# santi-pdp/segan_pytorch

Measured on NVIDIA H100. Metric: 16384-sample windows/sec (G+D train step), higher is better.
Workload: dtype f16 operands / f32 accumulate (f16 gradient tensors, loss scale 1024)

## Files before the change

### segan_pytorch_b200/csrc/tapgemm_tc.cu

```cuda
#include "common.cuh"
#include <cuda.h>
#include <stdlib.h>

namespace sg {

__device__ __forceinline__ uint32_t smem_u32(const void* p) {
  return static_cast<uint32_t>(__cvta_generic_to_shared(p));
}
__device__ __forceinline__ void mbar_init(uint64_t* bar, uint32_t count) {
  asm volatile("mbarrier.init.shared::cta.b64 [%0], %1;" ::"r"(smem_u32(bar)), "r"(count));
}
__device__ __forceinline__ void mbar_expect_tx(uint64_t* bar, uint32_t bytes) {
  asm volatile("mbarrier.arrive.expect_tx.shared::cta.b64 _, [%0], %1;" ::"r"(smem_u32(bar)), "r"(bytes)
               : "memory");
}
__device__ __forceinline__ void mbar_arrive(uint64_t* bar) {
  asm volatile("mbarrier.arrive.shared::cta.b64 _, [%0];" ::"r"(smem_u32(bar)) : "memory");
}
__device__ __forceinline__ uint32_t mbar_try(uint32_t addr, uint32_t parity) {
  uint32_t done;
  asm volatile(
      "{\n"
      ".reg .pred p;\n"
      "mbarrier.try_wait.parity.shared::cta.b64 p, [%1], %2;\n"
// ... 37 lines not shown
  asm volatile("prefetch.tensormap [%0];" ::"l"(reinterpret_cast<uint64_t>(map)) : "memory");
}
__device__ __forceinline__ void tma_store_3d(const CUtensorMap* map, uint32_t src, int c0, int c1, int c2) {
  asm volatile("cp.async.bulk.tensor.3d.global.shared::cta.bulk_group [%0, {%2, %3, %4}], [%1];"
               ::"l"(reinterpret_cast<uint64_t>(map)), "r"(src), "r"(c0), "r"(c1), "r"(c2)
               : "memory");
}
__device__ __forceinline__ void bulk_commit() { asm volatile("cp.async.bulk.commit_group;" ::: "memory"); }
__device__ __forceinline__ void bulk_wait_read_all() { asm volatile("cp.async.bulk.wait_group.read 0;" ::: "memory"); }
template <int N>
__device__ __forceinline__ void bulk_wait_read() { asm volatile("cp.async.bulk.wait_group.read %0;" ::"n"(N) : "memory"); }
__device__ __forceinline__ void fence_proxy_async_smem() { asm volatile("fence.proxy.async.shared::cta;" ::: "memory"); }
__device__ __forceinline__ void st_shared_u32(uint32_t addr, uint32_t v) {
  asm volatile("st.shared.b32 [%0], %1;" ::"r"(addr), "r"(v) : "memory");
}
__device__ __forceinline__ uint4 ld_shared_v4(uint32_t addr) {
  uint4 v;
  asm volatile("ld.shared.v4.b32 {%0, %1, %2, %3}, [%4];" : "=r"(v.x), "=r"(v.y), "=r"(v.z), "=r"(v.w) : "r"(addr) : "memory");
  return v;
}
__device__ __forceinline__ void red_add_v2(float* addr, float a, float b) {
  asm volatile("red.global.add.v2.f32 [%0], {%1, %2};" ::"l"(addr), "f"(a), "f"(b) : "memory");
}
__device__ __forceinline__ void wgmma_fence() { asm volatile("wgmma.fence.sync.aligned;" ::: "memory"); }
__device__ __forceinline__ void wgmma_commit() { asm volatile("wgmma.commit_group.sync.aligned;" ::: "memory"); }
template <int N>
__device__ __forceinline__ void wgmma_wait() { asm volatile("wgmma.wait_group.sync.aligned %0;" ::"n"(N) : "memory"); }
template <int R>
__device__ __forceinline__ void setmaxnreg_inc() { asm volatile("setmaxnreg.inc.sync.aligned.u32 %0;" ::"n"(R)); }
template <int R>
// ... 86 lines not shown

template <int N, int TA, int TB, bool BF16>
__device__ __forceinline__ void mma_k64(float (&acc)[N / 2], uint64_t da, uint64_t db, uint32_t a_step,
                                        uint32_t b_step, bool first) {
  wgmma_fence();
#pragma unroll
  for (int kk = 0; kk < 4; ++kk)
    wgmma_tile<N, TA, TB, BF16>(acc, da + kk * a_step, db + kk * b_step, (first && kk == 0) ? 0 : 1);
  wgmma_commit();
}

constexpr int STAGES = 4;
constexpr int A_STAGE_BYTES = 128 * 128;
constexpr int B_STAGE_BYTES = 256 * 128;
constexpr int STAGE_BYTES = A_STAGE_BYTES + B_STAGE_BYTES;
constexpr int SMEM_BYTES = STAGES * STAGE_BYTES + 1024  + 256  + 2048 ;
constexpr int SMEM_OPTIN_LIMIT = 232448;
constexpr int OUT_CHUNK_BYTES = 128 * 128;
template <int TN>
struct FSmem {
  static constexpr int RING = 4;
  static constexpr int STAGE_BYTES = A_STAGE_BYTES + TN * 128;
  static constexpr int BUFS = TN == 64 ? 2 : 1;
  static constexpr int BUF_BYTES = (TN == 256 ? 2 : 4) * OUT_CHUNK_BYTES / BUFS;
  static constexpr int STG_OFF = RING * STAGE_BYTES;
  static constexpr int CTL_OFF = STG_OFF + BUFS * BUF_BYTES;
  static constexpr int BYTES = CTL_OFF + 256  + 1024 ;
  static_assert(RING <= STAGES && STAGE_BYTES % 1024 == 0 && BUFS * BUF_BYTES >= 2048, "form-F shared memory");
};
static_assert(FSmem<64>::BYTES <= SMEM_OPTIN_LIMIT, "form-F TN 64 shared memory exceeds the sm_90 opt-in limit");
static_assert(FSmem<128>::BYTES <= SMEM_OPTIN_LIMIT, "form-F TN 128 shared memory exceeds the sm_90 opt-in limit");
static_assert(FSmem<256>::BYTES <= SMEM_OPTIN_LIMIT, "form-F TN 256 shared memory exceeds the sm_90 opt-in limit");
constexpr int NUM_THREADS = 384;
constexpr int PRODUCER_REGS = 40, CONSUMER_REGS = 232;

struct TapRangesTC {
  int k_lo[NTAP], k_hi[NTAP], n_lo[NTAP], n_hi[NTAP];
};

struct FTcParams {
  int a0_c, kc, nc, a_halo;
  int d_lo, d_hi;
  TapRangesTC tr;
// ... 114 lines not shown
    t.m_rel = 0;
    t.m0 = p.m_lo1;
    t.TR = p.TR1; t.TB = p.TB1; t.seg = 1;
  }
  return t;
}

__device__ __forceinline__ int f_mod(int x, int mod, int mask) { return mask >= 0 ? (x & mask) : (x % mod); }

__device__ __forceinline__ uint32_t pack2(float x, float y, int dtype) {
  if (dtype == SG_F16) return pack_half2_sat(x, y);
  __nv_bfloat162 h = __floats2bfloat162_rn(x, y);
  return *reinterpret_cast<uint32_t*>(&h);
}

__device__ __forceinline__ void f_store2(const FTcParams& p, float& x, float& y, int64_t o, int n_abs, bool atomic,
                                         int64_t o2, int64_t o2mirror) {
  if (p.out_dtype == SG_F32) {
    float* dst = reinterpret_cast<float*>(p.out) + o;
    if (atomic) red_add_v2(dst, x, y);
    else *reinterpret_cast<float2*>(dst) = make_float2(x, y);
    return;
  }
  float s0 = 0.f, s1 = 0.f;
  if (p.slope != nullptr) {
    const float* sp = p.slope + f_mod(n_abs, p.slope_mod, p.slope_mask);
    s0 = __ldg(sp); s1 = __ldg(sp + 1);
    if (p.out2 == nullptr) {
      x = x > 0.f ? x : s0 * x;
      y = y > 0.f ? y : s1 * y;
    }
  }
  *reinterpret_cast<uint32_t*>(reinterpret_cast<uint16_t*>(p.out) + o) = pack2(x, y, p.out_dtype);
  if (p.out2 != nullptr) {
    const uint32_t a = pack2(x > 0.f ? x : s0 * x, y > 0.f ? y : s1 * y, p.out_dtype);
    *reinterpret_cast<uint32_t*>(reinterpret_cast<uint16_t*>(p.out2) + o2) = a;
    if (o2mirror >= 0) *reinterpret_cast<uint32_t*>(reinterpret_cast<uint16_t*>(p.out2) + o2mirror) = a;
  }
}

__device__ __forceinline__ float round_as_stored(float x, int dtype) {
  if (dtype == SG_F16) return __half2float(__float2half_rn(x));
  if (dtype == SG_BF16) return __bfloat162float(__float2bfloat16_rn(x));
  return x;
}

template <int TN>
__device__ __forceinline__ void f_epilogue(const FTcParams& p, float (&acc)[TN / 2], const FTile& t, int n0, int ks,
                                           int ctid, float* colstat) {
  const int lane = ctid & 31, cw = ctid >> 5;
  const int out_buf_rows = p.out_rows + 2 * p.out_halo;
  const int out2_buf_rows = p.out_rows + 2 * p.out2_halo;
  const int col0 = n0 - p.n_lo + p.out_col0 + 2 * (lane & 3);
  int64_t obase[2], o2base[2], o2mirror[2];
  bool valid[2];
#pragma unroll
  for (int h = 0; h < 2; ++h) {
    const int r = cw * 16 + (lane >> 2) + 8 * h;
    const int tb = r / t.TR, tr = r - tb * t.TR;
    const int b = t.b0 + tb, m = t.m0 + tr;
    valid[h] = (tb < t.TB) && (b < p.batch) && (m < p.m_hi);
    obase[h] = ((int64_t)b * out_buf_rows + (m + p.out_halo)) * p.out_ld + col0;
    o2base[h] = 0; o2mirror[h] = -1;
    if (p.out2 != nullptr) {
      const int64_t rb = (int64_t)b * out2_buf_rows + p.out2_halo;
      o2base[h] = (rb + m) * p.out_ld + col0;
      if (p.out2_halo > 0) {
        int mm = 0;
        bool has = false;
        if (m >= 1 && m <= p.out2_halo) { mm = -m; has = true; }
        else if (m >= p.out_rows - 1 - p.out2_halo && m <= p.out_rows - 2) { mm = 2 * (p.out_rows - 1) - m; has = true; }
        if (has) o2mirror[h] = (rb + mm) * p.out_ld + col0;
      }
    }
  }
  const bool add_bias = p.bias != nullptr && ks == 0;
  const bool atomic = p.ksplit > 1;
#pragma unroll
  for (int j = 0; j < TN / 8; ++j) {
    const int c = 8 * j + 2 * (lane & 3);
    float bx = 0.f, by = 0.f;
    if (add_bias) {
      const float* bp = p.bias + f_mod(n0 + c, p.bias_mod, p.bias_mask);
      bx = __ldg(bp); by = __ldg(bp + 1);
    }
    float sx = 0.f, sy = 0.f, qx = 0.f, qy = 0.f;
#pragma unroll
    for (int h = 0; h < 2; ++h) {
      float x = acc[4 * j + 2 * h] + bx, y = acc[4 * j + 2 * h + 1] + by;
      if (valid[h]) {
        f_store2(p, x, y, obase[h] + 8 * j, n0 + c, atomic, o2base[h] + 8 * j, o2mirror[h] >= 0 ? o2mirror[h] + 8 * j : -1);
        x = round_as_stored(x, p.out_dtype);
        y = round_as_stored(y, p.out_dtype);
        sx += x; sy += y; qx += x * x; qy += y * y;
      }
    }
    if (p.stats != nullptr) {
#pragma unroll
      for (int o = 4; o < 32; o <<= 1) {
        sx += __shfl_xor_sync(0xffffffffu, sx, o);
        sy += __shfl_xor_sync(0xffffffffu, sy, o);
        qx += __shfl_xor_sync(0xffffffffu, qx, o);
        qy += __shfl_xor_sync(0xffffffffu, qy, o);
      }
      if (lane < 4) {
        atomicAdd(colstat + c, sx);
        atomicAdd(colstat + c + 1, sy);
        atomicAdd(colstat + 256 + c, qx);
        atomicAdd(colstat + 256 + c + 1, qy);
      }
    }
  }
}

template <bool F16>
__device__ __forceinline__ uint32_t pack2_t(float x, float y) {
  if constexpr (F16) return pack_half2_sat(x, y);
  __nv_bfloat162 h = __floats2bfloat162_rn(x, y);
  return *reinterpret_cast<uint32_t*>(&h);
}

template <int TN, bool F16, int MODE>
__device__ __forceinline__ void f_epilogue_tma_body(const FTcParams& p, const float (&acc)[TN / 2], const FTile& t,
                                                    int n0, int ctid, uint32_t buf, const CUtensorMap* tmO,
                                                    const CUtensorMap* tmO2) {
  constexpr bool two = MODE == 2;
  constexpr bool act_in_place = MODE == 1;
  const int lane = ctid & 31, cw = ctid >> 5;
  const int b0 = t.b0, m0 = t.m0;
  const bool add_bias = p.bias != nullptr;
  const uint32_t row_off = (uint32_t)(cw * 16 + (lane >> 2)) * 128u + 4u * (lane & 3);
  const int sw = lane >> 2;
  const int halo2 = p.out2_halo;
  const bool mirror_tile = two && halo2 > 0 &&
                           ((m0 <= halo2 && m0 + t.TR > 1) || (m0 + t.TR > p.out_rows - 1 - halo2 && m0 <= p.out_rows - 2));
  constexpr int NQ = TN / 64;
  constexpr int CH = FSmem<TN>::BUF_BYTES / OUT_CHUNK_BYTES;
  constexpr int QPR = two ? CH / 2 : CH;
  const int c_rel = n0 - p.n_lo, m_rel = t.m_rel;
#pragma unroll
// ... 30 lines not shown
        if constexpr (two) st_shared_u32(slot + OUT_CHUNK_BYTES + off, pack2_t<F16>(x > 0.f ? x : s0 * x, y > 0.f ? y : s1 * y));
      }
    }
    if (qi != QPR - 1 && q != NQ - 1) continue;
    fence_proxy_async_smem();
    consumer_bar_sync();
    if (ctid == 0) {
#pragma unroll
      for (int k = 0; k <= qi; ++k) {
        const uint32_t src = buf + (uint32_t)(two ? 2 * k : k) * OUT_CHUNK_BYTES;
        const int cq = c_rel + 64 * (q - qi + k);
        tma_store_3d(tmO, src, cq, m_rel, b0);
        if constexpr (two) tma_store_3d(tmO2, src + OUT_CHUNK_BYTES, cq, m_rel, b0);
      }
      bulk_commit();
    }
    if (mirror_tile) {
      const int rows = t.TR * t.TB;
      const int out2_buf_rows = p.out_rows + 2 * halo2;
      for (int idx = ctid; idx < rows * 8 * (qi + 1); idx += 256) {
        const int k = idx / (rows * 8), rk = idx - k * rows * 8;
        const int r = rk >> 3, kb = rk & 7;
        const int tb = r / t.TR, tr = r - tb * t.TR;
        const int b = b0 + tb, m = m0 + tr;
        if (b >= p.batch || m >= p.m_hi) continue;
        int mm;
        if (m >= 1 && m <= halo2) mm = -m;
        else if (m >= p.out_rows - 1 - halo2 && m <= p.out_rows - 2) mm = 2 * (p.out_rows - 1) - m;
        else continue;
        const uint32_t src = buf + (uint32_t)(2 * k + 1) * OUT_CHUNK_BYTES;
        const uint4 v = ld_shared_v4(src + (uint32_t)r * 128u + (uint32_t)((kb ^ (r & 7)) << 4));
        const int64_t o = ((int64_t)b * out2_buf_rows + halo2 + mm) * p.out_ld + p.out_col0 + c_rel +
                          64 * (q - qi + k) + 8 * kb;
        *reinterpret_cast<uint4*>(reinterpret_cast<uint16_t*>(p.out2) + o) = v;
      }
    }
  }
}

template <int TN>
__device__ __forceinline__ void f_epilogue_tma(const FTcParams& p, const float (&acc)[TN / 2], const FTile& t, int n0,
                                               int ctid, uint32_t buf, const CUtensorMap* tmO,
                                               const CUtensorMap* tmO2) {
  const int mode = p.out2 != nullptr ? 2 : (p.slope != nullptr ? 1 : 0);
  if (p.out_dtype == SG_F16) {
    if (mode == 2) f_epilogue_tma_body<TN, true, 2>(p, acc, t, n0, ctid, buf, tmO, tmO2);
    else if (mode == 1) f_epilogue_tma_body<TN, true, 1>(p, acc, t, n0, ctid, buf, tmO, tmO2);
    else f_epilogue_tma_body<TN, true, 0>(p, acc, t, n0, ctid, buf, tmO, tmO2);
  } else {
    if (mode == 2) f_epilogue_tma_body<TN, false, 2>(p, acc, t, n0, ctid, buf, tmO, tmO2);
    else if (mode == 1) f_epilogue_tma_body<TN, false, 1>(p, acc, t, n0, ctid, buf, tmO, tmO2);
    else f_epilogue_tma_body<TN, false, 0>(p, acc, t, n0, ctid, buf, tmO, tmO2);
  }
}

template <int TN, bool BF16>
__global__ void __launch_bounds__(NUM_THREADS, 1)
tapgemm_f_tc(const __grid_constant__ CUtensorMap tmA0, const __grid_constant__ CUtensorMap tmA1,
             const __grid_constant__ CUtensorMap tmW, const __grid_constant__ CUtensorMap tmO,
             const __grid_constant__ CUtensorMap tmO2, const __grid_constant__ CUtensorMap tmA0s1,
             const __grid_constant__ CUtensorMap tmA1s1, const __grid_constant__ CUtensorMap tmOs1,
             const FTcParams p) {
  extern __shared__ uint8_t smem_raw[];
  uint8_t* smem = reinterpret_cast<uint8_t*>((reinterpret_cast<uintptr_t>(smem_raw) + 1023) & ~uintptr_t(1023));
  using L = FSmem<TN>;
  SharedCtl* ctl = reinterpret_cast<SharedCtl*>(smem + L::CTL_OFF);
  float* colstat = reinterpret_cast<float*>(smem + L::STG_OFF);
  const int wg = threadIdx.x >> 7;

  if (threadIdx.x == 0) {
    prefetch_tmap(&tmA0); prefetch_tmap(&tmA1); prefetch_tmap(&tmW);
    if (p.tma_out) {
      prefetch_tmap(&tmO);
      if (p.out2 != nullptr) prefetch_tmap(&tmO2);
    }
    if (p.TR1 > 0) {
      prefetch_tmap(&tmA0s1); prefetch_tmap(&tmA1s1);
      if (p.tma_out) prefetch_tmap(&tmOs1);
    }
    for (int s = 0; s < L::RING; ++s) { mbar_init(&ctl->full[s], 1); mbar_init(&ctl->empty[s], 2); }
    fence_barrier_init();
  }
  if (p.stats != nullptr)
    for (int c = threadIdx.x; c < 512; c += NUM_THREADS) colstat[c] = 0.f;
  __syncthreads();

  const int total_tiles = p.m_tiles * p.n_tiles * p.ksplit;
  const uint32_t b_bytes = (uint32_t)TN * 128u;
  PieceIter it;
  it.init(p, p.m_tiles, total_tiles, blockIdx.x, gridDim.x);
  Piece pc;

  if (wg == 0) {
    setmaxnreg_dec<PRODUCER_REGS>();
    if (threadIdx.x == 0) {
      int stage = 0; uint32_t phase = 0;
      while (it.next(p, pc)) {
        const int ks = p.ksplit == 1 ? 0 : pc.rest % p.ksplit;
        const int nt = p.ksplit == 1 ? pc.rest : pc.rest / p.ksplit;
// ... 38 lines not shown
          }
          step += nk;
        }
      }
    }
    return;
  }

  setmaxnreg_inc<CONSUMER_REGS>();
  const int ctid = threadIdx.x - 128;
  const int cwg = wg - 1;
  const bool wg_leader = (threadIdx.x & 127) == 0;
  const uint32_t smem0 = smem_u32(smem);
  int stage = 0; uint32_t phase = 0;
  int stat_nt = -1;
  auto flush_stats = [&](int nt_done) {
    consumer_bar_sync();
    const int n0s = p.n_lo + nt_done * p.TN;
    double* o = p.stats + (int64_t)(blockIdx.x % SG_STAT_SLICES) * 2 * p.nc;
    for (int c = ctid; c < p.TN; c += 256) {
      atomicAdd(o + n0s + c, (double)colstat[c]);
      atomicAdd(o + p.nc + n0s + c, (double)colstat[256 + c]);
      colstat[c] = 0.f;
      colstat[256 + c] = 0.f;
    }
    consumer_bar_sync();
  };
  const bool tl_on = (p.dbg & (1 << 20)) && ctid == 0 && blockIdx.x < TL_CTAS;
  int tl_i = 0;
  unsigned long long* tl = g_tc_timeline + (blockIdx.x < TL_CTAS ? blockIdx.x : 0) * TL_SLOTS;
  if (tl_on) { for (int i = 0; i < TL_SLOTS; ++i) tl[i] = 0; tl[tl_i++] = gtime_ns(); }

  int staged = 0;
  float acc[TN / 2];
  while (it.next(p, pc)) {
    const int ks = p.ksplit == 1 ? 0 : pc.rest % p.ksplit;
    const int nt = p.ksplit == 1 ? pc.rest : pc.rest / p.ksplit;
    const int n0 = p.n_lo + nt * p.TN;
    const bool partial = pc.tile >= it.dp_end;
    if (p.stats != nullptr && nt != stat_nt) {
      if (stat_nt >= 0) flush_stats(stat_nt);
      stat_nt = nt;
    }
    const int nsteps = pc.ke - pc.kb;
    if (nsteps == 0) {
#pragma unroll
      for (int j = 0; j < TN / 2; ++j) acc[j] = 0.f;
    }
    int prev = 0;
    for (int i = 0; i < nsteps; ++i) {
      mbar_wait(&ctl->full[stage], phase);
      const uint32_t sa = smem0 + (uint32_t)stage * L::STAGE_BYTES;
      mma_k64<TN, 0, 0, BF16>(acc, make_smem_desc(sa + (uint32_t)cwg * 8192u, 16, 1024),
                        make_smem_desc(sa + A_STAGE_BYTES, 16, 1024), 2, 2, i == 0);
      wgmma_wait<1>();
      if (i > 0 && wg_leader) mbar_arrive(&ctl->empty[prev]);
      prev = stage;
      if (++stage == L::RING) { stage = 0; phase ^= 1; }
    }
    wgmma_wait<0>();
    if (nsteps > 0 && wg_leader) mbar_arrive(&ctl->empty[prev]);
    if (tl_on && tl_i < TL_SLOTS - 1) tl[tl_i++] = gtime_ns();

    if (!partial) {
      if (p.tma_out) {
        const uint32_t buf = smem0 + L::STG_OFF + (uint32_t)(staged++ % L::BUFS) * L::BUF_BYTES;
        const FTile t = f_tile(p, pc.mt);
        f_epilogue_tma<TN>(p, acc, t, n0, ctid, buf, t.seg ? &tmOs1 : &tmO, &tmO2);
      } else f_epilogue<TN>(p, acc, f_tile(p, pc.mt), n0, ks, ctid, colstat);
      if (tl_on && tl_i < TL_SLOTS - 1) tl[tl_i++] = gtime_ns();
      continue;
    }
    constexpr int64_t SLOT_F2 = 128 * 256 / 2;
    float2* myslot = reinterpret_cast<float2*>(p.sk_ws) + (int64_t)blockIdx.x * SLOT_F2 + ctid;
#pragma unroll
    for (int j = 0; j < TN / 4; ++j) __stcg(myslot + j * 256, make_float2(acc[2 * j], acc[2 * j + 1]));
    if (tl_on && tl_i < TL_SLOTS - 1) tl[tl_i++] = gtime_ns();
    const int slot = pc.tile - it.dp_end;
    unsigned int* cnt = p.sk_cnt + slot * 8 + (ctid >> 5);
    __threadfence();
    __syncwarp();
    unsigned int old = 0;
    if ((ctid & 31) == 0) old = atomicAdd(cnt, 1u);
    old = __shfl_sync(0xffffffffu, old, 0);
    if (old + 1u == (unsigned int)p.sk_split) {
      __threadfence();
#pragma unroll
      for (int j = 0; j < TN / 2; ++j) acc[j] = 0.f;
      const float2* base0 = reinterpret_cast<const float2*>(p.sk_ws) + (int64_t)slot * p.sk_split * SLOT_F2 + ctid;
      for (int sp = 0; sp < p.sk_split; ++sp) {
#pragma unroll
        for (int j = 0; j < TN / 4; ++j) {
          const float2 t = __ldcg(base0 + sp * SLOT_F2 + j * 256);
          acc[2 * j] += t.x; acc[2 * j + 1] += t.y;
        }
      }
      f_epilogue<TN>(p, acc, f_tile(p, pc.mt), n0, 0, ctid, colstat);
      __syncwarp();
      if ((ctid & 31) == 0) *cnt = 0u;
      if (tl_on && tl_i < TL_SLOTS - 1) tl[tl_i++] = gtime_ns() | (1ull << 63);
    }
  }
  if (tl_on && tl_i < TL_SLOTS) tl[tl_i++] = gtime_ns();
  if (p.stats != nullptr && stat_nt >= 0) flush_stats(stat_nt);
  if (p.tma_out && ctid == 0) bulk_wait_read_all();
}

struct WTcParams {
  int a0_c, kc, nc, a_halo;
  int d_lo, d_hi;
  TapRangesTC tr;
  float* dw; int dw_tap0;
  int g_rows, batch, ksplit;
  int PR, PB;
  int n_tiles, k_tiles;
  int row_chunks, b_chunks;
  const float* out_scale;
};

// ... 197 lines not shown
static int num_sms() {
  static int n = 0;
  if (n == 0) {
    int dev = 0;
    cudaGetDevice(&dev);
    cudaDeviceGetAttribute(&n, cudaDevAttrMultiProcessorCount, dev);
    if (n <= 0) n = NUM_SMS;
  }
  return n;
}

template <typename K>
static int launch_persistent(K kern, int grid, const CUtensorMap& t0, const CUtensorMap& t1, const CUtensorMap& t2,
                             const void* params, cudaStream_t st);

int tapgemm_f_tc_launch(const sg_tapgemm_f* q, cudaStream_t st) {
  FTcParams p;
  p.a0_c = q->a0_c; p.kc = q->kc; p.nc = q->nc; p.a_halo = q->a_halo;
  p.d_lo = q->d_lo; p.d_hi = q->d_hi;
  for (int i = 0; i < NTAP; ++i) {
    p.tr.k_lo[i] = q->tap_k_lo[i]; p.tr.k_hi[i] = q->tap_k_hi[i];
    p.tr.n_lo[i] = q->tap_n_lo[i]; p.tr.n_hi[i] = q->tap_n_hi[i];
  }
  p.out = q->out; p.out_dtype = q->out_dtype; p.out_rows = q->out_rows; p.out_halo = q->out_halo;
  p.out_ld = q->out_ld > 0 ? q->out_ld : q->nc;
  p.out_col0 = q->out_ld > 0 ? q->out_col0 : q->n_lo;
  p.w_tap0 = q->w_tap0;
  p.m_lo = q->m_lo; p.m_hi = q->m_hi; p.n_lo = q->n_lo;
  p.bias = q->bias; p.bias_mod = q->bias_mod > 0 ? q->bias_mod : q->nc;
  p.batch = q->batch; p.ksplit = q->ksplit < 1 ? 1 : q->ksplit;
  const int rows_m = q->m_hi - q->m_lo;
  const int ncols = q->n_hi - q->n_lo;
  p.TN = (ncols % 256 == 0) ? 256 : (ncols % 128 == 0 ? 128 : 64);
  if ((q->tile_n == 64 || q->tile_n == 128 || q->tile_n == 256) && ncols % q->tile_n == 0 && q->tile_n < p.TN)
    p.TN = q->tile_n;
  p.n_tiles = ncols / p.TN;
  auto seg_tiles = [&](int R, int& TR, int& TB) {
    if (R >= 128) { TR = 128; TB = 1; }
    else { TR = R; TB = 128 / R; if (TB > q->batch) TB = q->batch; }
    return ((R + TR - 1) / TR) * ((q->batch + TB - 1) / TB);
  };
  int R0 = rows_m;
  p.m_tiles0 = seg_tiles(rows_m, p.TR, p.TB);
  p.m_tiles = p.m_tiles0;
  p.m_lo1 = q->m_hi; p.TR1 = 0; p.TB1 = 0;
  if (q->out2 == nullptr && q->bn_stats == nullptr) {
    int r0 = 128 * (rows_m / 128);
    if (rows_m <= 128) for (r0 = 1; 2 * r0 <= rows_m; r0 *= 2) {}
    if (r0 < rows_m) {
      int TR0, TB0, TR1, TB1;
      const int t0 = seg_tiles(r0, TR0, TB0), t1 = seg_tiles(rows_m - r0, TR1, TB1);
      if (t0 + t1 < p.m_tiles && (t0 + t1) * p.n_tiles * p.ksplit >= num_sms()) {
        R0 = r0;
        p.TR = TR0; p.TB = TB0; p.m_tiles0 = t0; p.m_tiles = t0 + t1;
        p.m_lo1 = q->m_lo + r0; p.TR1 = TR1; p.TB1 = TB1;
      }
    }
  }
  p.m_tiles_per_b = (R0 + p.TR - 1) / p.TR;
  static const bool verbose = getenv("SEGAN_B200_SK_VERBOSE") != nullptr;
  if (verbose)
// ... 17 lines not shown
  else tmA1 = tmA0;
  if (rc) return rc;
  CUtensorMap tmA0s1 = tmA0, tmA1s1 = tmA1;
  if (p.TR1 > 0) {
    rc = make_map3(&tmA0s1, q->a0, q->a_dtype, q->a0_c, a_buf_rows, q->batch, p.TR1, p.TB1);
    if (rc) return rc;
    if (q->a1) rc = make_map3(&tmA1s1, q->a1, q->a_dtype, q->a1_c, a_buf_rows, q->batch, p.TR1, p.TB1);
    else tmA1s1 = tmA0s1;
    if (rc) return rc;
  }
  rc = make_map2(&tmW, q->w, q->w_dtype, q->kc, (int64_t)(q->d_hi + 4 - q->w_tap0 + 1) * q->nc, p.TN);
  if (rc) return rc;
  const int tiles = p.m_tiles * p.n_tiles * p.ksplit;
  int nctas = num_sms();
  if (tiles < nctas) nctas = tiles;
  if (q->sk_ws != nullptr && g_stream_k > 1 && p.ksplit == 1 && q->bn_stats == nullptr && nctas <= SK_MAX_CTAS &&
      tiles > nctas && tiles % nctas != 0) {
    const int r = tiles % nctas;
    int steps = 0;
    for (int d = q->d_lo; d <= q->d_hi; ++d) steps += (q->tap_k_hi[d + 4] - q->tap_k_lo[d + 4]) / 64;
    int best_s = 1;
    double best = (double)steps;
    int s_max = nctas / r < g_stream_k ? nctas / r : g_stream_k;
    if (s_max > steps / 2) s_max = steps / 2;
    const double per_partial = g_sk_atomic_steps * 256.0 / p.TN;
    for (int S = 2; S <= s_max; ++S) {
      const double c = (double)steps / S + per_partial * S + g_sk_fixed_steps;
      if (c < best) { best = c; best_s = S; }
    }
    const bool split = best_s > 1 && best < 0.92 * steps && steps >= 2 * best_s;
    if (verbose)
      fprintf(stderr, "tapgemm_f split-K: %d tiles on %d CTAs, %d left over, %d k-steps, TN %d -> split %d\n",
              tiles, nctas, r, steps, p.TN, split ? best_s : 1);
    if (split) {
      p.sk_dp_tiles = (tiles / nctas) * nctas;
      p.sk_split = best_s;
      p.sk_cnt = reinterpret_cast<unsigned int*>(q->sk_ws);
      p.sk_ws = reinterpret_cast<float*>(reinterpret_cast<uint8_t*>(q->sk_ws) + SK_CNT_BYTES);
    }
  }
  p.tma_out = q->out_dtype != SG_F32 && q->bn_stats == nullptr;
  CUtensorMap tmO = tmA0, tmO2 = tmA0, tmOs1 = tmA0;
  if (p.tma_out) {
    rc = make_store_map3(&tmO, q->out, q->out_dtype, ncols, R0, q->batch, p.out_ld, q->out_rows + 2 * q->out_halo,
                         q->out_halo + q->m_lo, p.out_col0, p.TR, p.TB);
    if (rc) return rc;
    if (p.TR1 > 0) {
      rc = make_store_map3(&tmOs1, q->out, q->out_dtype, ncols, rows_m - R0, q->batch, p.out_ld,
                           q->out_rows + 2 * q->out_halo, q->out_halo + p.m_lo1, p.out_col0, p.TR1, p.TB1);
      if (rc) return rc;
    }
    if (q->out2 != nullptr) {
      rc = make_store_map3(&tmO2, q->out2, q->out_dtype, ncols, rows_m, q->batch, p.out_ld,
                           q->out_rows + 2 * q->out2_halo, q->out2_halo + q->m_lo, p.out_col0, p.TR, p.TB);
      if (rc) return rc;
    }
  }
  const bool bf = q->a_dtype == SG_BF16;
  void (*kern)(CUtensorMap, CUtensorMap, CUtensorMap, CUtensorMap, CUtensorMap, CUtensorMap, CUtensorMap, CUtensorMap,
               FTcParams);
  int smem_bytes;
  if (p.TN == 256) { kern = bf ? tapgemm_f_tc<256, true> : tapgemm_f_tc<256, false>; smem_bytes = FSmem<256>::BYTES; }
  else if (p.TN == 128) { kern = bf ? tapgemm_f_tc<128, true> : tapgemm_f_tc<128, false>; smem_bytes = FSmem<128>::BYTES; }
  else { kern = bf ? tapgemm_f_tc<64, true> : tapgemm_f_tc<64, false>; smem_bytes = FSmem<64>::BYTES; }
  SG_CHECK_CUDA(cudaFuncSetAttribute(kern, cudaFuncAttributeMaxDynamicSharedMemorySize, smem_bytes));
  void* args[] = {&tmA0, &tmA1, &tmW, &tmO, &tmO2, &tmA0s1, &tmA1s1, &tmOs1, &p};
  SG_CHECK_CUDA(cudaLaunchKernel(reinterpret_cast<const void*>(kern), dim3(nctas), dim3(NUM_THREADS), args,
                                 (size_t)smem_bytes, st));
  return SG_OK;
}

template <typename K>
static int launch_persistent(K kern, int grid, const CUtensorMap& t0, const CUtensorMap& t1, const CUtensorMap& t2,
                             const void* params, cudaStream_t st) {
  SG_CHECK_CUDA(cudaFuncSetAttribute(kern, cudaFuncAttributeMaxDynamicSharedMemorySize, SMEM_BYTES));
  void* args[] = {const_cast<CUtensorMap*>(&t0), const_cast<CUtensorMap*>(&t1), const_cast<CUtensorMap*>(&t2),
                  const_cast<void*>(params)};
  SG_CHECK_CUDA(cudaLaunchKernel(reinterpret_cast<const void*>(kern), dim3(grid), dim3(NUM_THREADS), args,
                                 (size_t)SMEM_BYTES, st));
// ... 42 lines not shown
```

### segan_pytorch_b200/engine.py

```python
import ctypes as C
import math
import os

import torch

from . import _lib
from ._lib import (ACT_NONE, ACT_PRELU, BACKEND_FFMA, BACKEND_TCGEN05, SG_BF16, SG_DHEAD_CONV, SG_DHEAD_GAVG,
                   SG_DHEAD_GMAX, SG_DHEAD_MLP, SG_F16, SG_F32, TapGemmF, TapGemmW)

KW_MIN, KW_MAX = 4, 32


def kwidth_served(k):
    return isinstance(k, int) and not isinstance(k, bool) and KW_MIN <= k <= KW_MAX


def conv_offset(k):
    return k // 2 - 1


def deconv_padding(k):
    return max(0, (4 - k) // -2)


# ... 145 lines not shown
    def __enter__(self):
        if PROFILE is not None:
            self.s = torch.cuda.Event(enable_timing=True)
            self.e = torch.cuda.Event(enable_timing=True)
            self.s.record()
        return self

    def __exit__(self, *a):
        if PROFILE is not None:
            self.e.record()
            PROFILE.append((self.kind, self.s, self.e, self.flops))
        return False


NUM_SMS = 132
FUSE_BN_STATS = os.environ.get("SEGAN_B200_FUSE_BN_STATS", "0").lower() not in ("0", "off", "no", "false")
SPLIT_WAVES = os.environ.get("SEGAN_B200_WAVE_SPLIT", "0").lower() not in ("0", "off", "no", "false")


def _f_tiling(rows_m, batch, ncols, tile_n=0):
    if rows_m >= 128:
        tb, mpb = 1, (rows_m + 127) // 128
    else:
        tb, mpb = max(1, min(128 // rows_m, batch, 256)), 1
    tn = 256 if ncols % 256 == 0 else (128 if ncols % 128 == 0 else 64)
    if tile_n in (64, 128, 256) and ncols % tile_n == 0 and tile_n < tn:
        tn = tile_n
    m_tiles = mpb * ((batch + tb - 1) // tb)
    tiles = ((m_tiles + 1) // 2) * (ncols // tn)
    gran = 2 * tb if mpb % 2 else tb
    return tb, mpb, tn, tiles, gran
# ... 1352 lines not shown
        x1 = x1.contiguous().float()
        Lq = [L // 4 ** (l + 1) for l in range(nl)]
        if self.pool_type == "none":
            assert Lq[-1] * fm[-1] == self._param("fc.0.weight" + self.wsfx).shape[1], "D expects L = 16384"
        elif self.pool_type == "conv":
            assert Lq[-1] == self._param("fc.weight" + self.wsfx).shape[1], "D expects L = 4^n_layers * pool_slen"
        if shifts_dev is not None and not wave_on_tensor_cores():
            raise _lib.SeganB200Error("device-resident phase shifts need the tensor-core waveform route")

        def rptr(i):
            return None if shifts_dev is None else C.c_void_p(shifts_dev.data_ptr() + 4 * i)
        a, hp, ss, mi, hpb = [None] * nl, [None] * nl, [None] * nl, [None] * nl, [None] * nl
        bnorm = not self.snorm
        stats = stat_arena(buf, "d.stats", [(SL, 2, fm[l]) for l in range(nl)], dev) if (training and bnorm) else None
        eff_backend = default_backend() if self.backend is None else self.backend
        fuse_stats = (training and bnorm and FUSE_BN_STATS and eff_backend == BACKEND_TCGEN05 and B * Lq[-1] >= 256)
        for l in range(nl):
            cout = fm[l]
            a[l] = buf.get("d.a%d" % l, (B, Lq[l], cout), F16, dev)
            bias = self.pview("enc_blocks.%d.conv.bias" % l) if m.bias else None
            colb = None
            if l == 0 and wave_on_tensor_cores():
                col16 = buf.get("d.col16", (B, Lq[0], 64), F16, dev)
                colb0 = buf.get("d.colb", (B, Lq[0], 64), GT, dev) if twins else None
                _lib.call("sg_wave_im2col_kw", _p(x0), _p(x1), 2, B, L, int(shifts[0]), rptr(0), 1, conv_offset(self.kw),
                          self.kw, _p(col16), _p(colb0), st)
                if alias:
                    colb0 = col16
                self.wait_packed("small")
                run_f(col16, None, Lq[0], 0, SG_F16, self.packed["Wcol0"], SG_F16, 64, 64,
                      tap_ranges("full", 0, 64, 64), a[0], SG_F16, Lq[0], 0, 0, Lq[0], B, bias=bias, bias_mod=64,
                      d_lo=0, d_hi=0, w_tap0=4, backend=self.backend, stats=stats[0] if fuse_stats else None)
            elif l == 0:
                colb0 = None
                w0 = self.pview("enc_blocks.0.conv.weight" + self.wsfx)
                if self.snorm:
                    w0 = (w0 * self.sn_inv_sigma("enc_blocks.0.conv.weight_orig")).contiguous()
                _lib.call("sg_wave_conv_fwd", _p(x0), _p(x1), 2, B, L, int(shifts[0]),
                          _p(w0), _p(bias), cout, _p(a[0]), None, None, st)
            else:
                cin = fm[l - 1]
                self.wait_packed("Wf%d" % l)
                taps = tap_ranges("conv_fwd", cin, 4 * cin, cout, self.kw)
                d_lo, d_hi = tap_span(taps)
                run_f(hp[l - 1], None, Lq[l], 4, SG_F16, self.packed["Wf%d" % l], SG_F16, 4 * cin, cout,
                      taps, a[l], SG_F16, Lq[l], 0, 0, Lq[l], B, d_lo=d_lo, d_hi=d_hi,
                      bias=bias, bias_mod=cout, backend=self.backend, stats=stats[l] if fuse_stats else None)
            bn = m.enc_blocks[l].norm
            if bnorm:
                ss[l] = buf.get("d.ss%d" % l, (2, cout), F32, dev)
                mi[l] = buf.get("d.mi%d" % l, (2, cout), F32, dev)
            if not bnorm:
                pass
            elif training:
                st2 = stats[l]
                if not (fuse_stats and (l > 0 or wave_on_tensor_cores())):
                    _lib.call("sg_bn_stats", _p(a[l]), SG_F16, B * Lq[l], cout, _p(st2), st)
                _lib.call("sg_bn_finalize", _p(st2), B * Lq[l], cout,
                          _p(self.pview("enc_blocks.%d.norm.weight" % l)),
                          _p(self.pview("enc_blocks.%d.norm.bias" % l)), self.eps, self.momentum,
                          _p(bn.running_mean), _p(bn.running_var), _p(ss[l]), _p(mi[l]), st)
                bn.num_batches_tracked += 1
            else:
                invstd = torch.rsqrt(bn.running_var + self.eps)
                sc = self.pview("enc_blocks.%d.norm.weight" % l) * invstd
                ss[l][0].copy_(sc)
                ss[l][1].copy_(self.pview("enc_blocks.%d.norm.bias" % l) - bn.running_mean * sc)
                mi[l][0].copy_(bn.running_mean)
                mi[l][1].copy_(invstd)
            halo = 16 if l < nl - 1 else 0
            roll = int(shifts[l + 1]) if l < nl - 1 else 0
# ... 323 lines not shown
```

Measured before the change: 11120.

## Fuse BatchNorm statistics into TMA-store GEMM epilogue with register accumulation

Reworks fused BN stats in the tap-GEMM kernel. Per-column sums now accumulate in registers, read back from the staged f16/bf16 output tile in shared memory, and are flushed with double atomics per warp. This replaces the shared-memory colstat array and its block barriers, and lets stats-producing launches keep the TMA store path, stream-K and segment splitting. The Python side enables fusion by default per layer (except channel counts divisible by 256), dropping the separate sg_bn_stats pass. The cost is extra registers, more template instantiations, and more global atomic traffic.

```diff
diff --git a/segan_pytorch_b200/csrc/tapgemm_tc.cu b/segan_pytorch_b200/csrc/tapgemm_tc.cu
--- a/segan_pytorch_b200/csrc/tapgemm_tc.cu
+++ b/segan_pytorch_b200/csrc/tapgemm_tc.cu
@@ -75,6 +75,11 @@
 __device__ __forceinline__ void st_shared_u32(uint32_t addr, uint32_t v) {
   asm volatile("st.shared.b32 [%0], %1;" ::"r"(addr), "r"(v) : "memory");
 }
+__device__ __forceinline__ uint32_t ld_shared_u32(uint32_t addr) {
+  uint32_t v;
+  asm volatile("ld.shared.b32 %0, [%1];" : "=r"(v) : "r"(addr) : "memory");
+  return v;
+}
 __device__ __forceinline__ uint4 ld_shared_v4(uint32_t addr) {
   uint4 v;
   asm volatile("ld.shared.v4.b32 {%0, %1, %2, %3}, [%4];" : "=r"(v.x), "=r"(v.y), "=r"(v.z), "=r"(v.w) : "r"(addr) : "memory");
@@ -191,7 +196,7 @@
 constexpr int A_STAGE_BYTES = 128 * 128;
 constexpr int B_STAGE_BYTES = 256 * 128;
 constexpr int STAGE_BYTES = A_STAGE_BYTES + B_STAGE_BYTES;
-constexpr int SMEM_BYTES = STAGES * STAGE_BYTES + 1024  + 256  + 2048 ;
+constexpr int SMEM_BYTES = STAGES * STAGE_BYTES + 1024  + 256 ;
 constexpr int SMEM_OPTIN_LIMIT = 232448;
 constexpr int OUT_CHUNK_BYTES = 128 * 128;
 template <int TN>
@@ -203,7 +208,7 @@
   static constexpr int STG_OFF = RING * STAGE_BYTES;
   static constexpr int CTL_OFF = STG_OFF + BUFS * BUF_BYTES;
   static constexpr int BYTES = CTL_OFF + 256  + 1024 ;
-  static_assert(RING <= STAGES && STAGE_BYTES % 1024 == 0 && BUFS * BUF_BYTES >= 2048, "form-F shared memory");
+  static_assert(RING <= STAGES && STAGE_BYTES % 1024 == 0, "form-F shared memory");
 };
 static_assert(FSmem<64>::BYTES <= SMEM_OPTIN_LIMIT, "form-F TN 64 shared memory exceeds the sm_90 opt-in limit");
 static_assert(FSmem<128>::BYTES <= SMEM_OPTIN_LIMIT, "form-F TN 128 shared memory exceeds the sm_90 opt-in limit");
@@ -348,7 +353,7 @@
   return *reinterpret_cast<uint32_t*>(&h);
 }
 
-__device__ __forceinline__ void f_store2(const FTcParams& p, float& x, float& y, int64_t o, int n_abs, bool atomic,
+__device__ __forceinline__ void f_store2(const FTcParams& p, float x, float y, int64_t o, int n_abs, bool atomic,
                                          int64_t o2, int64_t o2mirror) {
   if (p.out_dtype == SG_F32) {
     float* dst = reinterpret_cast<float*>(p.out) + o;
@@ -373,15 +378,103 @@
   }
 }
 
-__device__ __forceinline__ float round_as_stored(float x, int dtype) {
-  if (dtype == SG_F16) return __half2float(__float2half_rn(x));
-  if (dtype == SG_BF16) return __bfloat162float(__float2bfloat16_rn(x));
-  return x;
+template <bool F16>
+__device__ __forceinline__ uint32_t pack2_t(float x, float y) {
+  if constexpr (F16) return pack_half2_sat(x, y);
+  __nv_bfloat162 h = __floats2bfloat162_rn(x, y);
+  return *reinterpret_cast<uint32_t*>(&h);
+}
+template <bool F16>
+__device__ __forceinline__ float2 unpack2_t(uint32_t w) {
+  if constexpr (F16) return __half22float2(*reinterpret_cast<const __half2*>(&w));
+  return make_float2(__uint_as_float(w << 16), __uint_as_float(w & 0xffff0000u));
+}
+
+__device__ __forceinline__ double* stat_slice(const FTcParams& p, int n0, int lane) {
+  const int slice = (blockIdx.x + (threadIdx.x >> 5)) % SG_STAT_SLICES;
+  return p.stats + (int64_t)slice * 2 * p.nc + n0 + 8 * (lane >> 2) + 2 * (lane & 3);
+}
+
+template <bool F16, typename Word>
+__device__ __forceinline__ void stat_pair(const bool (&live)[2], Word word, int jj, float (&v)[4]) {
+  v[0] = v[1] = v[2] = v[3] = 0.f;
+#pragma unroll
+  for (int h = 0; h < 2; ++h) {
+    if (live[h]) {
+      const float2 f = unpack2_t<F16>(word(jj, h));
+      v[0] += f.x; v[1] += f.y;
+      v[2] = fmaf(f.x, f.x, v[2]); v[3] = fmaf(f.y, f.y, v[3]);
+    }
+  }
+}
+
+template <int TN>
+struct StatRegs {
+  static constexpr int N = TN == 64 ? 32 : TN / 16;
+};
+
+__device__ __forceinline__ void stat_reduce(const float (&v)[32], int lane, float (&t)[4]) {
+  float w[16], u[8];
+  const bool k4 = lane & 16, k3 = lane & 8, k2 = lane & 4;
+#pragma unroll
+  for (int i = 0; i < 16; ++i)
+    w[i] = (k4 ? v[i + 16] : v[i]) + __shfl_xor_sync(0xffffffffu, k4 ? v[i] : v[i + 16], 16);
+#pragma unroll
+  for (int i = 0; i < 8; ++i) u[i] = (k3 ? w[i + 8] : w[i]) + __shfl_xor_sync(0xffffffffu, k3 ? w[i] : w[i + 8], 8);
+#pragma unroll
+  for (int i = 0; i < 4; ++i) t[i] = (k2 ? u[i + 4] : u[i]) + __shfl_xor_sync(0xffffffffu, k2 ? u[i] : u[i + 4], 4);
+}
+
+template <int TN, bool F16, typename Word>
+__device__ __forceinline__ void stat_words(const bool (&live)[2], Word word, float (&own)[StatRegs<TN>::N], int q,
+                                           int lane) {
+  float v[32];
+#pragma unroll
+  for (int jj = 0; jj < 8; ++jj) {
+    float p4[4];
+    stat_pair<F16>(live, word, jj, p4);
+#pragma unroll
+    for (int s = 0; s < 4; ++s) {
+      if constexpr (TN == 64) own[4 * jj + s] += p4[s];
+      else v[4 * jj + s] = p4[s];
+    }
+  }
+  if constexpr (TN != 64) {
+    float t[4];
+    stat_reduce(v, lane, t);
+#pragma unroll
+    for (int i = 0; i < 4; ++i) own[4 * q + i] += t[i];
+  }
+}
+
+template <int TN>
+__device__ __forceinline__ void stat_flush(const FTcParams& p, float (&own)[StatRegs<TN>::N], int n0, int lane) {
+  double* o = stat_slice(p, n0, lane);
+  if constexpr (TN == 64) {
+    float t[4];
+    stat_reduce(own, lane, t);
+#pragma unroll
+    for (int s = 0; s < 4; ++s) atomicAdd(o + (s >> 1) * p.nc + (s & 1), (double)t[s]);
+  } else {
+#pragma unroll
+    for (int q = 0; q < TN / 64; ++q) {
+#pragma unroll
+      for (int s = 0; s < 4; ++s) atomicAdd(o + (s >> 1) * p.nc + 64 * q + (s & 1), (double)own[4 * q + s]);
+    }
+  }
+#pragma unroll
+  for (int i = 0; i < StatRegs<TN>::N; ++i) own[i] = 0.f;
+}
+
+__device__ __forceinline__ bool f_row(const FTcParams& p, const FTile& t, int r, int& b, int& m) {
+  const int tb = r / t.TR, tr = r - tb * t.TR;
+  b = t.b0 + tb; m = t.m0 + tr;
+  return (tb < t.TB) && (b < p.batch) && (m < p.m_hi);
 }
 
 template <int TN>
 __device__ __forceinline__ void f_epilogue(const FTcParams& p, float (&acc)[TN / 2], const FTile& t, int n0, int ks,
-                                           int ctid, float* colstat) {
+                                           int ctid) {
   const int lane = ctid & 31, cw = ctid >> 5;
   const int out_buf_rows = p.out_rows + 2 * p.out_halo;
   const int out2_buf_rows = p.out_rows + 2 * p.out2_halo;
@@ -390,10 +483,8 @@
   bool valid[2];
 #pragma unroll
   for (int h = 0; h < 2; ++h) {
-    const int r = cw * 16 + (lane >> 2) + 8 * h;
-    const int tb = r / t.TR, tr = r - tb * t.TR;
-    const int b = t.b0 + tb, m = t.m0 + tr;
-    valid[h] = (tb < t.TB) && (b < p.batch) && (m < p.m_hi);
+    int b, m;
+    valid[h] = f_row(p, t, cw * 16 + (lane >> 2) + 8 * h, b, m);
     obase[h] = ((int64_t)b * out_buf_rows + (m + p.out_halo)) * p.out_ld + col0;
     o2base[h] = 0; o2mirror[h] = -1;
     if (p.out2 != nullptr) {
@@ -418,46 +509,38 @@
       const float* bp = p.bias + f_mod(n0 + c, p.bias_mod, p.bias_mask);
       bx = __ldg(bp); by = __ldg(bp + 1);
     }
-    float sx = 0.f, sy = 0.f, qx = 0.f, qy = 0.f;
 #pragma unroll
     for (int h = 0; h < 2; ++h) {
-      float x = acc[4 * j + 2 * h] + bx, y = acc[4 * j + 2 * h + 1] + by;
-      if (valid[h]) {
+      const float x = acc[4 * j + 2 * h] + bx, y = acc[4 * j + 2 * h + 1] + by;
+      if (valid[h])
         f_store2(p, x, y, obase[h] + 8 * j, n0 + c, atomic, o2base[h] + 8 * j, o2mirror[h] >= 0 ? o2mirror[h] + 8 * j : -1);
-        x = round_as_stored(x, p.out_dtype);
-        y = round_as_stored(y, p.out_dtype);
-        sx += x; sy += y; qx += x * x; qy += y * y;
-      }
-    }
-    if (p.stats != nullptr) {
-#pragma unroll
-      for (int o = 4; o < 32; o <<= 1) {
-        sx += __shfl_xor_sync(0xffffffffu, sx, o);
-        sy += __shfl_xor_sync(0xffffffffu, sy, o);
-        qx += __shfl_xor_sync(0xffffffffu, qx, o);
-        qy += __shfl_xor_sync(0xffffffffu, qy, o);
-      }
-      if (lane < 4) {
-        atomicAdd(colstat + c, sx);
-        atomicAdd(colstat + c + 1, sy);
-        atomicAdd(colstat + 256 + c, qx);
-        atomicAdd(colstat + 256 + c + 1, qy);
-      }
-    }
-  }
-}
-
-template <bool F16>
-__device__ __forceinline__ uint32_t pack2_t(float x, float y) {
-  if constexpr (F16) return pack_half2_sat(x, y);
-  __nv_bfloat162 h = __floats2bfloat162_rn(x, y);
-  return *reinterpret_cast<uint32_t*>(&h);
-}
-
-template <int TN, bool F16, int MODE>
+    }
+  }
+}
+
+template <int TN, bool F16>
+__device__ __forceinline__ void f_stats_from_out(const FTcParams& p, const FTile& t, int n0, int ctid,
+                                                 float (&own)[StatRegs<TN>::N]) {
+  const int lane = ctid & 31, cw = ctid >> 5;
+  const uint32_t* row[2];
+  bool live[2];
+#pragma unroll
+  for (int h = 0; h < 2; ++h) {
+    int b, m;
+    live[h] = f_row(p, t, cw * 16 + (lane >> 2) + 8 * h, b, m);
+    row[h] = reinterpret_cast<const uint32_t*>(reinterpret_cast<const uint16_t*>(p.out) +
+        ((int64_t)b * (p.out_rows + 2 * p.out_halo) + (m + p.out_halo)) * p.out_ld + n0 - p.n_lo + p.out_col0 +
+        2 * (lane & 3));
+  }
+#pragma unroll
+  for (int q = 0; q < TN / 64; ++q)
+    stat_words<TN, F16>(live, [&](int jj, int h) { return row[h][32 * q + 4 * jj]; }, own, q, lane);
+}
+
+template <int TN, bool F16, int MODE, bool STATS>
 __device__ __forceinline__ void f_epilogue_tma_body(const FTcParams& p, const float (&acc)[TN / 2], const FTile& t,
                                                     int n0, int ctid, uint32_t buf, const CUtensorMap* tmO,
-                                                    const CUtensorMap* tmO2) {
+                                                    const CUtensorMap* tmO2, float (&own)[StatRegs<TN>::N]) {
   constexpr bool two = MODE == 2;
   constexpr bool act_in_place = MODE == 1;
   const int lane = ctid & 31, cw = ctid >> 5;
@@ -518,6 +601,21 @@
         if constexpr (two) tma_store_3d(tmO2, src + OUT_CHUNK_BYTES, cq, m_rel, b0);
       }
       bulk_commit();
+    }
+    if constexpr (STATS) {
+      bool live[2];
+#pragma unroll
+      for (int h = 0; h < 2; ++h) {
+        int b, m;
+        live[h] = f_row(p, t, cw * 16 + (lane >> 2) + 8 * h, b, m);
+      }
+#pragma unroll
+      for (int k = 0; k <= qi; ++k) {
+        const uint32_t src = buf + (uint32_t)(two ? 2 * k : k) * OUT_CHUNK_BYTES + row_off;
+        stat_words<TN, F16>(live, [&](int jj, int h) {
+          return ld_shared_u32(src + (uint32_t)h * 1024u + (uint32_t)((jj ^ sw) << 4));
+        }, own, q - qi + k, lane);
+      }
     }
     if (mirror_tile) {
       const int rows = t.TR * t.TB;
@@ -542,23 +640,24 @@
   }
 }
 
-template <int TN>
+template <int TN, bool F16, bool STATS>
+__device__ __forceinline__ void f_epilogue_tma_mode(const FTcParams& p, const float (&acc)[TN / 2], const FTile& t,
+                                                    int n0, int ctid, uint32_t buf, const CUtensorMap* tmO,
+                                                    const CUtensorMap* tmO2, float (&own)[StatRegs<TN>::N]) {
+  if (p.out2 != nullptr) f_epilogue_tma_body<TN, F16, 2, STATS>(p, acc, t, n0, ctid, buf, tmO, tmO2, own);
+  else if (p.slope != nullptr) f_epilogue_tma_body<TN, F16, 1, STATS>(p, acc, t, n0, ctid, buf, tmO, tmO2, own);
+  else f_epilogue_tma_body<TN, F16, 0, STATS>(p, acc, t, n0, ctid, buf, tmO, tmO2, own);
+}
+
+template <int TN, bool STATS>
 __device__ __forceinline__ void f_epilogue_tma(const FTcParams& p, const float (&acc)[TN / 2], const FTile& t, int n0,
                                                int ctid, uint32_t buf, const CUtensorMap* tmO,
-                                               const CUtensorMap* tmO2) {
-  const int mode = p.out2 != nullptr ? 2 : (p.slope != nullptr ? 1 : 0);
-  if (p.out_dtype == SG_F16) {
-    if (mode == 2) f_epilogue_tma_body<TN, true, 2>(p, acc, t, n0, ctid, buf, tmO, tmO2);
-    else if (mode == 1) f_epilogue_tma_body<TN, true, 1>(p, acc, t, n0, ctid, buf, tmO, tmO2);
-    else f_epilogue_tma_body<TN, true, 0>(p, acc, t, n0, ctid, buf, tmO, tmO2);
-  } else {
-    if (mode == 2) f_epilogue_tma_body<TN, false, 2>(p, acc, t, n0, ctid, buf, tmO, tmO2);
-    else if (mode == 1) f_epilogue_tma_body<TN, false, 1>(p, acc, t, n0, ctid, buf, tmO, tmO2);
-    else f_epilogue_tma_body<TN, false, 0>(p, acc, t, n0, ctid, buf, tmO, tmO2);
-  }
-}
-
-template <int TN, bool BF16>
+                                               const CUtensorMap* tmO2, float (&own)[StatRegs<TN>::N]) {
+  if (p.out_dtype == SG_F16) f_epilogue_tma_mode<TN, true, STATS>(p, acc, t, n0, ctid, buf, tmO, tmO2, own);
+  else f_epilogue_tma_mode<TN, false, STATS>(p, acc, t, n0, ctid, buf, tmO, tmO2, own);
+}
+
+template <int TN, bool BF16, bool STATS>
 __global__ void __launch_bounds__(NUM_THREADS, 1)
 tapgemm_f_tc(const __grid_constant__ CUtensorMap tmA0, const __grid_constant__ CUtensorMap tmA1,
              const __grid_constant__ CUtensorMap tmW, const __grid_constant__ CUtensorMap tmO,
@@ -569,7 +668,6 @@
   uint8_t* smem = reinterpret_cast<uint8_t*>((reinterpret_cast<uintptr_t>(smem_raw) + 1023) & ~uintptr_t(1023));
   using L = FSmem<TN>;
   SharedCtl* ctl = reinterpret_cast<SharedCtl*>(smem + L::CTL_OFF);
-  float* colstat = reinterpret_cast<float*>(smem + L::STG_OFF);
   const int wg = threadIdx.x >> 7;
 
   if (threadIdx.x == 0) {
@@ -585,8 +683,6 @@
     for (int s = 0; s < L::RING; ++s) { mbar_init(&ctl->full[s], 1); mbar_init(&ctl->empty[s], 2); }
     fence_barrier_init();
   }
-  if (p.stats != nullptr)
-    for (int c = threadIdx.x; c < 512; c += NUM_THREADS) colstat[c] = 0.f;
   __syncthreads();
 
   const int total_tiles = p.m_tiles * p.n_tiles * p.ksplit;
@@ -655,18 +751,9 @@
   const uint32_t smem0 = smem_u32(smem);
   int stage = 0; uint32_t phase = 0;
   int stat_nt = -1;
-  auto flush_stats = [&](int nt_done) {
-    consumer_bar_sync();
-    const int n0s = p.n_lo + nt_done * p.TN;
-    double* o = p.stats + (int64_t)(blockIdx.x % SG_STAT_SLICES) * 2 * p.nc;
-    for (int c = ctid; c < p.TN; c += 256) {
-      atomicAdd(o + n0s + c, (double)colstat[c]);
-      atomicAdd(o + p.nc + n0s + c, (double)colstat[256 + c]);
-      colstat[c] = 0.f;
-      colstat[256 + c] = 0.f;
-    }
-    consumer_bar_sync();
-  };
+  float own[StatRegs<TN>::N];
+#pragma unroll
+  for (int i = 0; i < StatRegs<TN>::N; ++i) own[i] = 0.f;
   const bool tl_on = (p.dbg & (1 << 20)) && ctid == 0 && blockIdx.x < TL_CTAS;
   int tl_i = 0;
   unsigned long long* tl = g_tc_timeline + (blockIdx.x < TL_CTAS ? blockIdx.x : 0) * TL_SLOTS;
@@ -679,8 +766,8 @@
     const int nt = p.ksplit == 1 ? pc.rest : pc.rest / p.ksplit;
     const int n0 = p.n_lo + nt * p.TN;
     const bool partial = pc.tile >= it.dp_end;
-    if (p.stats != nullptr && nt != stat_nt) {
-      if (stat_nt >= 0) flush_stats(stat_nt);
+    if (STATS && nt != stat_nt) {
+      if (stat_nt >= 0) stat_flush<TN>(p, own, p.n_lo + stat_nt * p.TN, ctid & 31);
       stat_nt = nt;
     }
     const int nsteps = pc.ke - pc.kb;
@@ -707,8 +794,8 @@
       if (p.tma_out) {
         const uint32_t buf = smem0 + L::STG_OFF + (uint32_t)(staged++ % L::BUFS) * L::BUF_BYTES;
         const FTile t = f_tile(p, pc.mt);
-        f_epilogue_tma<TN>(p, acc, t, n0, ctid, buf, t.seg ? &tmOs1 : &tmO, &tmO2);
-      } else f_epilogue<TN>(p, acc, f_tile(p, pc.mt), n0, ks, ctid, colstat);
+        f_epilogue_tma<TN, STATS>(p, acc, t, n0, ctid, buf, t.seg ? &tmOs1 : &tmO, &tmO2, own);
+      } else f_epilogue<TN>(p, acc, f_tile(p, pc.mt), n0, ks, ctid);
       if (tl_on && tl_i < TL_SLOTS - 1) tl[tl_i++] = gtime_ns();
       continue;
     }
@@ -736,14 +823,19 @@
           acc[2 * j] += t.x; acc[2 * j + 1] += t.y;
         }
       }
-      f_epilogue<TN>(p, acc, f_tile(p, pc.mt), n0, 0, ctid, colstat);
+      const FTile t = f_tile(p, pc.mt);
+      f_epilogue<TN>(p, acc, t, n0, 0, ctid);
+      if constexpr (STATS) {
+        if (p.out_dtype == SG_F16) f_stats_from_out<TN, true>(p, t, n0, ctid, own);
+        else f_stats_from_out<TN, false>(p, t, n0, ctid, own);
+      }
       __syncwarp();
       if ((ctid & 31) == 0) *cnt = 0u;
       if (tl_on && tl_i < TL_SLOTS - 1) tl[tl_i++] = gtime_ns() | (1ull << 63);
     }
   }
   if (tl_on && tl_i < TL_SLOTS) tl[tl_i++] = gtime_ns();
-  if (p.stats != nullptr && stat_nt >= 0) flush_stats(stat_nt);
+  if (STATS && stat_nt >= 0) stat_flush<TN>(p, own, p.n_lo + stat_nt * p.TN, ctid & 31);
   if (p.tma_out && ctid == 0) bulk_wait_read_all();
 }
 
@@ -971,6 +1063,14 @@
 static int launch_persistent(K kern, int grid, const CUtensorMap& t0, const CUtensorMap& t1, const CUtensorMap& t2,
                              const void* params, cudaStream_t st);
 
+typedef void (*FKern)(CUtensorMap, CUtensorMap, CUtensorMap, CUtensorMap, CUtensorMap, CUtensorMap, CUtensorMap,
+                      CUtensorMap, FTcParams);
+template <int TN>
+static FKern f_kernel(bool bf, bool stats) {
+  if (bf) return stats ? tapgemm_f_tc<TN, true, true> : tapgemm_f_tc<TN, true, false>;
+  return stats ? tapgemm_f_tc<TN, false, true> : tapgemm_f_tc<TN, false, false>;
+}
+
 int tapgemm_f_tc_launch(const sg_tapgemm_f* q, cudaStream_t st) {
   FTcParams p;
   p.a0_c = q->a0_c; p.kc = q->kc; p.nc = q->nc; p.a_halo = q->a_halo;
@@ -1001,7 +1101,7 @@
   p.m_tiles0 = seg_tiles(rows_m, p.TR, p.TB);
   p.m_tiles = p.m_tiles0;
   p.m_lo1 = q->m_hi; p.TR1 = 0; p.TB1 = 0;
-  if (q->out2 == nullptr && q->bn_stats == nullptr) {
+  if (q->out2 == nullptr) {
     int r0 = 128 * (rows_m / 128);
     if (rows_m <= 128) for (r0 = 1; 2 * r0 <= rows_m; r0 *= 2) {}
     if (r0 < rows_m) {
@@ -1049,7 +1149,7 @@
   const int tiles = p.m_tiles * p.n_tiles * p.ksplit;
   int nctas = num_sms();
   if (tiles < nctas) nctas = tiles;
-  if (q->sk_ws != nullptr && g_stream_k > 1 && p.ksplit == 1 && q->bn_stats == nullptr && nctas <= SK_MAX_CTAS &&
+  if (q->sk_ws != nullptr && g_stream_k > 1 && p.ksplit == 1 && nctas <= SK_MAX_CTAS &&
       tiles > nctas && tiles % nctas != 0) {
     const int r = tiles % nctas;
     int steps = 0;
@@ -1074,7 +1174,7 @@
       p.sk_ws = reinterpret_cast<float*>(reinterpret_cast<uint8_t*>(q->sk_ws) + SK_CNT_BYTES);
     }
   }
-  p.tma_out = q->out_dtype != SG_F32 && q->bn_stats == nullptr;
+  p.tma_out = q->out_dtype != SG_F32;
   CUtensorMap tmO = tmA0, tmO2 = tmA0, tmOs1 = tmA0;
   if (p.tma_out) {
     rc = make_store_map3(&tmO, q->out, q->out_dtype, ncols, R0, q->batch, p.out_ld, q->out_rows + 2 * q->out_halo,
@@ -1091,13 +1191,12 @@
       if (rc) return rc;
     }
   }
-  const bool bf = q->a_dtype == SG_BF16;
-  void (*kern)(CUtensorMap, CUtensorMap, CUtensorMap, CUtensorMap, CUtensorMap, CUtensorMap, CUtensorMap, CUtensorMap,
-               FTcParams);
+  const bool bf = q->a_dtype == SG_BF16, stats = q->bn_stats != nullptr;
+  FKern kern;
   int smem_bytes;
-  if (p.TN == 256) { kern = bf ? tapgemm_f_tc<256, true> : tapgemm_f_tc<256, false>; smem_bytes = FSmem<256>::BYTES; }
-  else if (p.TN == 128) { kern = bf ? tapgemm_f_tc<128, true> : tapgemm_f_tc<128, false>; smem_bytes = FSmem<128>::BYTES; }
-  else { kern = bf ? tapgemm_f_tc<64, true> : tapgemm_f_tc<64, false>; smem_bytes = FSmem<64>::BYTES; }
+  if (p.TN == 256) { kern = f_kernel<256>(bf, stats); smem_bytes = FSmem<256>::BYTES; }
+  else if (p.TN == 128) { kern = f_kernel<128>(bf, stats); smem_bytes = FSmem<128>::BYTES; }
+  else { kern = f_kernel<64>(bf, stats); smem_bytes = FSmem<64>::BYTES; }
   SG_CHECK_CUDA(cudaFuncSetAttribute(kern, cudaFuncAttributeMaxDynamicSharedMemorySize, smem_bytes));
   void* args[] = {&tmA0, &tmA1, &tmW, &tmO, &tmO2, &tmA0s1, &tmA1s1, &tmOs1, &p};
   SG_CHECK_CUDA(cudaLaunchKernel(reinterpret_cast<const void*>(kern), dim3(nctas), dim3(NUM_THREADS), args,
diff --git a/segan_pytorch_b200/engine.py b/segan_pytorch_b200/engine.py
--- a/segan_pytorch_b200/engine.py
+++ b/segan_pytorch_b200/engine.py
@@ -183,7 +183,6 @@
 
 
 NUM_SMS = 132
-FUSE_BN_STATS = os.environ.get("SEGAN_B200_FUSE_BN_STATS", "0").lower() not in ("0", "off", "no", "false")
 SPLIT_WAVES = os.environ.get("SEGAN_B200_WAVE_SPLIT", "0").lower() not in ("0", "off", "no", "false")
 
 
@@ -1566,7 +1565,8 @@
         bnorm = not self.snorm
         stats = stat_arena(buf, "d.stats", [(SL, 2, fm[l]) for l in range(nl)], dev) if (training and bnorm) else None
         eff_backend = default_backend() if self.backend is None else self.backend
-        fuse_stats = (training and bnorm and FUSE_BN_STATS and eff_backend == BACKEND_TCGEN05 and B * Lq[-1] >= 256)
+        fuse = [training and bnorm and eff_backend == BACKEND_TCGEN05 and fm[l] % 256 != 0 and
+                (l > 0 or wave_on_tensor_cores()) for l in range(nl)]
         for l in range(nl):
             cout = fm[l]
             a[l] = buf.get("d.a%d" % l, (B, Lq[l], cout), F16, dev)
@@ -1582,7 +1582,7 @@
                 self.wait_packed("small")
                 run_f(col16, None, Lq[0], 0, SG_F16, self.packed["Wcol0"], SG_F16, 64, 64,
                       tap_ranges("full", 0, 64, 64), a[0], SG_F16, Lq[0], 0, 0, Lq[0], B, bias=bias, bias_mod=64,
-                      d_lo=0, d_hi=0, w_tap0=4, backend=self.backend, stats=stats[0] if fuse_stats else None)
+                      d_lo=0, d_hi=0, w_tap0=4, backend=self.backend, stats=stats[0] if fuse[0] else None)
             elif l == 0:
                 colb0 = None
                 w0 = self.pview("enc_blocks.0.conv.weight" + self.wsfx)
@@ -1597,7 +1597,7 @@
                 d_lo, d_hi = tap_span(taps)
                 run_f(hp[l - 1], None, Lq[l], 4, SG_F16, self.packed["Wf%d" % l], SG_F16, 4 * cin, cout,
                       taps, a[l], SG_F16, Lq[l], 0, 0, Lq[l], B, d_lo=d_lo, d_hi=d_hi,
-                      bias=bias, bias_mod=cout, backend=self.backend, stats=stats[l] if fuse_stats else None)
+                      bias=bias, bias_mod=cout, backend=self.backend, stats=stats[l] if fuse[l] else None)
             bn = m.enc_blocks[l].norm
             if bnorm:
                 ss[l] = buf.get("d.ss%d" % l, (2, cout), F32, dev)
@@ -1606,7 +1606,7 @@
                 pass
             elif training:
                 st2 = stats[l]
-                if not (fuse_stats and (l > 0 or wave_on_tensor_cores())):
+                if not fuse[l]:
                     _lib.call("sg_bn_stats", _p(a[l]), SG_F16, B * Lq[l], cout, _p(st2), st)
                 _lib.call("sg_bn_finalize", _p(st2), B * Lq[l], cout,
                           _p(self.pview("enc_blocks.%d.norm.weight" % l)),
```

Result: faster. 11270 (median of 6 runs) (+1.4%).
